# astra-vision/rain-rendering

Measured on AMD Instinct MI355X. Metric: rainy frames/sec @ 1242x375, 100 mm/hr, higher is better.
Workload: dtype f64 alpha/mask, f32 colour

## Files before the change

### rain-rendering_amd/csrc/rainhip.hip

```cpp
#include <hip/hip_runtime.h>

#include <dlfcn.h>

#include <cstddef>
#include <cstdio>
#include <cstdlib>
#include <algorithm>
#include <cstring>
#include <string>
#include <type_traits>
#include <mutex>
#include <unordered_map>
#include <vector>

#include "rainhip.h"
#include "rr_device.h"
#include "rr_prepass.h"
#include "rr_deflate.h"
#include "rr_pngrows.h"
#include "rr_particles.h"
#include "rr_lens.h"

using namespace rr;

// ... 555 lines not shown
    m = wrap ? N + 4 : N;
    int* qx = s_px[wave][g];
    int* qy = s_py[wave][g];
    const int idx = (wrap && k > pp) ? k + 4 : k;
    qx[idx] = ipx;
    qy[idx] = ipy;
    if (wrap && k == pp) {
      const int cols = dm.We, rows = dm.He;
      if (top) {
        qx[pp + 1] = cols; qy[pp + 1] = ipy;
        qx[pp + 2] = cols; qy[pp + 2] = 0;
        qx[pp + 3] = 0;    qy[pp + 3] = 0;
        qx[pp + 4] = 0;    qy[pp + 4] = ipy_next;
      } else {
        qx[pp + 1] = 0;    qy[pp + 1] = ipy;
        qx[pp + 2] = 0;    qy[pp + 2] = rows;
        qx[pp + 3] = cols; qy[pp + 3] = rows;
        qx[pp + 4] = cols; qy[pp + 4] = ipy_next;
      }
    }
  }
  if (ext) {
    const rr_ext_tile e = fr.ext[dg];
    const int np = imin(imax(e.n_poly, 0), POLY_STRIDE);
    bool fine = true;
    for (int v = k; v < np; v += N) {
      const double vx = e.poly_xy[2 * v], vy = e.poly_xy[2 * v + 1];
      fine = fine && fov_coord_ok(vx) && fov_coord_ok(vy);
      s_px[wave][g][v] = (int32_t)vx;
      s_py[wave][g][v] = (int32_t)vy;
    }
    const unsigned long long bad_e = __ballot(!fine) & gmask;
    m = bad_e ? 0 : np;
  }
  wave_lds_sync();
  {
    const int* qx = s_px[wave][imin(g, FOV_GROUPS - 1)];
    const int* qy = s_py[wave][imin(g, FOV_GROUPS - 1)];
    const int x0v = m > 0 ? qx[0] : 0, y0v = m > 0 ? qy[0] : 0;
    int vdif = -1;
    for (int v = k; v < m; v += N)
      if (vdif < 0 && (qx[v] != x0v || qy[v] != y0v)) vdif = v;
    const unsigned long long bd = __ballot(vdif >= 0) & gmask;
    const int va = __shfl(vdif, bd ? __ffsll((long long)bd) - 1 : lane);
    bool nz = false;
    if (bd) {
      const int64_t ax = (int64_t)qx[va] - x0v, ay = (int64_t)qy[va] - y0v;
      for (int v = k; v < m; v += N) nz = nz || (ax * ((int64_t)qy[v] - y0v) - ay * ((int64_t)qx[v] - x0v) != 0);
    }
    if ((__ballot(nz) & gmask) == 0ull) m = 0;
  }
  if (act && k == 0) sc.npts[gi] = m;
  const int He = dm.He;
  int* xl = s_xl[wave];
  int* xr = s_xr[wave];
  uint32_t packed[FOV_GROUPS][NCH];
#pragma unroll
  for (int c = 0; c < NCH; c++) {
    xl[c * 64 + lane] = 1 << 30;
    xr[c * 64 + lane] = -(1 << 30);
#pragma unroll
    for (int k = 0; k < FOV_GROUPS; k++) packed[k][c] = 0;
  }
  for (int gg = 0; gg < G; gg++) {
    const int mg = __builtin_amdgcn_readfirstlane(__shfl(m, gg * N));
    if (mg <= 0) continue;
    const bool cvg = cv_rule && fov_fill_rule_cv_applies(s_px[wave][gg], s_py[wave][gg], mg, N, He, dm.We);
    int cnt = 0;
    if (lane < mg) {
      const int j = (lane + 1 == mg) ? 0 : lane + 1;
      const int x0 = s_px[wave][gg][lane], y0 = s_py[wave][gg][lane], x1 = s_px[wave][gg][j], y1 = s_py[wave][gg][j];
      const bool swp = y1 < y0;
      const int ylo = swp ? y1 : y0, yhi = swp ? y0 : y1;
      const int xa = swp ? x1 : x0, dx = (swp ? x0 : x1) - xa;
      const int den = yhi - ylo;
      const float inv = den > 0 ? 1.0f / (float)(2 * den) : 0.f;
      const int ra = imax(ylo, 0), rb = imin(yhi, He - 1);
      cnt = rb - ra + 1;
      int d16 = 0, q_hh = 0, q_hr = 0;
      if (cvg && den > 0) edge_cv_consts(dx, den, d16, q_hh, q_hr);
      s_edge[wave][3 * lane] = make_int4(ylo, ra, rb, xa);
      s_edge[wave][3 * lane + 1] = make_int4(dx, den, __float_as_int(inv), 0);
      s_edge[wave][3 * lane + 2] = make_int4(d16, q_hh, q_hr, 0);
    }
    wave_lds_sync();
    for (int e = 0; e < mg; e += 2) {
      const int eb = imin(e + 1, mg - 1);
      const int nmax = imax(__builtin_amdgcn_readlane(cnt, e), __builtin_amdgcn_readlane(cnt, eb));
      if (nmax <= 0) continue;
      const int me = lane < 32 ? e : eb;
      const int4 A = s_edge[wave][3 * me], B = s_edge[wave][3 * me + 1], C = s_edge[wave][3 * me + 2];
      const int ylo = A.x, ra = A.y, rbv = A.z, xa = A.w, dx = B.x, den = B.y;
      const float inv = __int_as_float(B.z);
      const bool hz = den == 0;
      const int hz_l = imin(xa, xa + dx), hz_h = imax(xa, xa + dx);
      const int dx2 = 2 * dx, dn = 2 * den;
      for (int c = 0; c < nmax; c += 32) {
        const int y = ra + c + (lane & 31);
        if (y <= rbv) {
          const int t = y - ylo;
          const int n2 = __mul24(dx2, t);
          int q = (int)floorf((float)n2 * inv);
          int rem = n2 - __mul24(q, dn);
          if (rem < 0) { q -= 1; rem += dn; }
          else if (rem >= dn) { q += 1; rem -= dn; }
          int l = xa + q + (rem >= den ? 1 : 0), h = l;
          if (cvg && !hz) edge_row_cv(xa, xa + dx, den, dx, C.x, C.y, C.z, t, q, rem, l, h);
          atomicMin(&xl[y], hz ? hz_l : l);
          atomicMax(&xr[y], hz ? hz_h : h);
        }
      }
    }
    wave_lds_sync();
#pragma unroll
    for (int c = 0; c < NCH; c++) {
      const int y = c * 64 + lane;
      const int a = imax(xl[y], 0), b = imin(xr[y], dm.We - 1);
      xl[y] = 1 << 30;
      xr[y] = -(1 << 30);
      uint32_t v = 0;
      if (y < He && a <= b) v = (uint32_t)a | ((uint32_t)(b + 1) << 16);
#pragma unroll
      for (int k = 0; k < FOV_GROUPS; k++)
        if (k == gg) packed[k][c] = v;
    }
  }
  bool have[FOV_GROUPS];
  int dk[FOV_GROUPS];
  const int col = (from_list && act) ? sc.fov_slot[gi] : dg;
#pragma unroll
  for (int k = 0; k < FOV_GROUPS; k++) {
    have[k] = k < G && __builtin_amdgcn_readfirstlane(__shfl(m, k < G ? k * N : 0)) > 0;
    dk[k] = __builtin_amdgcn_readfirstlane(__shfl(col, k < G ? k * N : 0));
  }
#pragma unroll
  for (int c = 0; c < NCH; c++) {
    const int y = c * 64 + lane;
    if (y < Hp) {
      uint32_t* out = sc.spans + ((int64_t)f * Hp + y) * Dp;
#pragma unroll
      for (int k = 0; k < FOV_GROUPS; k++)
        if (have[k]) out[dk[k]] = packed[k][c];
    }
  }
  if (!from_list) break;
  wave_lds_sync();
  }
}

#ifndef RR_DDA_WAVES
#define RR_DDA_WAVES 1
#endif
constexpr int DDA_WAVES = RR_DDA_WAVES;
template <int CTRL, int ROW_MASK>
__device__ inline int dpp_keep_i32(int v) { return __builtin_amdgcn_update_dpp(v, v, CTRL, ROW_MASK, 0xf, false); }
__device__ inline int wave_min_scan_i32(int v) {
  v = imin(v, dpp_keep_i32<0x111, 0xf>(v));
  v = imin(v, dpp_keep_i32<0x112, 0xf>(v));
  v = imin(v, dpp_keep_i32<0x114, 0xf>(v));
  v = imin(v, dpp_keep_i32<0x118, 0xf>(v));
  v = imin(v, dpp_keep_i32<0x142, 0xa>(v));
  v = imin(v, dpp_keep_i32<0x143, 0xc>(v));
  return v;
}
__device__ inline int wave_max_scan_i32(int v) {
  v = imax(v, dpp_keep_i32<0x111, 0xf>(v));
  v = imax(v, dpp_keep_i32<0x112, 0xf>(v));
  v = imax(v, dpp_keep_i32<0x114, 0xf>(v));
  v = imax(v, dpp_keep_i32<0x118, 0xf>(v));
  v = imax(v, dpp_keep_i32<0x142, 0xa>(v));
  v = imax(v, dpp_keep_i32<0x143, 0xc>(v));
  return v;
}

constexpr uint32_t FOV_KEY_LAST = 0xffffu;
__global__ __launch_bounds__(64 * DDA_WAVES) void k_fov_vertices(const FrameDesc* frames, Dims dm, rr_camera cam, int max_drops, int ordered, Scratch sc) {
  const int f = blockIdx.y, wave = threadIdx.x >> 6, lane = threadIdx.x & 63;
  const FrameDesc& fr = frames[f];
  const int N = cam.n_fov;
  const int i = (blockIdx.x * DDA_WAVES + wave) * 64 + lane;
  const bool act = i < fr.n_drops;
  const int64_t gi = (int64_t)f * max_drops + (act ? i : 0);
  if (fr.strategy == 1) {
    if (act) {
      sc.npts[gi] = -1;
      sc.fov_rec[gi] = make_uint4(0u, 0u, 0u, (ordered ? FOV_KEY_LAST : 0u) << 16);
    }
    return;
  }
  uint32_t* const gpix = sc.fov_pix + (int64_t)f * N * max_drops + (act ? i : 0);
  auto pixv = [&](int kk) -> uint32_t& { return gpix[(int64_t)kk * max_drops]; };
  uint32_t top_xy = 0;
  int uns = 0;
  int count_true = 0, count_false = 0;
  int ktop = 0, ytop = 1 << 30, ybot = -(1 << 30), r_first = 0;
  bool spread = false, on_map = true;
  int turns = 0, dir = 0, dir_first = 0;
  float dist = 0.f;
  if (act) {
    FovSetup32 F;
    const rr_drop d = load_drop(fr.drops + i);
    fov_setup32(d, (float)cam.fov_cos, (float)cam.fov_sin, F, uns);
    dist = sqrtf(F.pos[0] * F.pos[0] + F.pos[1] * F.pos[1] + F.pos[2] * F.pos[2]);
    float az_prev = 0.f, er_prev = 0.f, az0 = 0.f, er0 = 0.f;
    int y_prev = 0, y0v = 0;
    for (int k = 0; k < N; k++) {
      float az, er, pxf, pyf;
      fov_vertex32(F, (float)cam.radius, (float)cam.phi_cos[k], (float)cam.phi_sin[k], dm.He, dm.We, az, er, pxf, pyf, uns);
      const int ix = (int)pxf, iy = (int)pyf;
      const uint32_t vxy = (uint32_t)(ix & 0xffff) | ((uint32_t)(iy & 0xffff) << 16);
      pixv(k) = vxy;
      on_map = on_map && ix >= 0 && ix < dm.We && iy >= 0 && iy < dm.He;
      const int r = imin(imax(iy, 0), dm.He - 1);
      if (k == 0) { az0 = az; er0 = er; r_first = r; y0v = iy; }
      else {
        const bool c = fov_wrap_cnd32(az_prev, az, er_prev, er, uns);
        count_true += c ? 1 : 0;
        count_false += c ? 0 : 1;
        spread = spread || iabs(r - r_first) >= 2;
        const int sg = iy > y_prev ? 1 : (iy < y_prev ? -1 : 0);
        if (sg != 0) {
          if (dir == 0) dir_first = sg;
          else if (sg != dir) turns++;
          dir = sg;
        }
      }
      if (iy < ytop) { ytop = iy; ktop = k; top_xy = vxy; }
      ybot = imax(ybot, iy);
      az_prev = az; er_prev = er; y_prev = iy;
    }
    {
      const bool c = fov_wrap_cnd32(az_prev, az0, er_prev, er0, uns);
      count_true += c ? 1 : 0;
      count_false += c ? 0 : 1;
      const int sg = y0v > y_prev ? 1 : (y0v < y_prev ? -1 : 0);
      if (sg != 0) {
        if (dir != 0 && sg != dir) turns++;
        dir = sg;
      }
      if (dir != 0 && dir_first != 0 && dir != dir_first) turns++;
    }
  }
  if (act) {
    const uint32_t v0 = pixv(0), va = pixv(N / 2);
    const int x0v = (int)(v0 & 0xffffu), y0v = (int)(v0 >> 16), ax = (int)(va & 0xffffu) - x0v, ay = (int)(va >> 16) - y0v;
    bool sure_nc = false;
    for (int k = 1; k < N; k++) {
      const uint32_t v = pixv(k);
      sure_nc = sure_nc || poly_surely_not_collinear_step(ax, ay, (int)(v & 0xffffu) - x0v, (int)(v >> 16) - y0v);
    }
    if (!sure_nc) uns |= 256;
  }
  const bool certain_fail = (uns & 128) && !(uns & 3);
  const bool wrap = count_true == 1 || count_false == 1;
  const bool undecided = (uns & ~128) != 0 || count_true == 0 || count_false == 0 || (!wrap && !spread);
  const bool monotone = turns <= 2;
  const bool mine = act && !certain_fail && !undecided && !wrap && monotone;
  if (act && certain_fail) sc.npts[gi] = 0;
  if (act && !certain_fail && !mine) {
    const int pos = atomicAdd(&sc.fov_list_n[f], 1);
    sc.fov_list[(int64_t)f * max_drops + pos] = i;
  }
  if (mine) sc.npts[gi] = N;
  if (act) {
    uint32_t key = 0u;
    if (ordered) {
      const int bucket = (int)fminf(fmaxf(dist * 4.0f, 0.f), 62.0f);
      key = mine ? ((uint32_t)bucket << 10) | (uint32_t)imin(imax(ytop, 0), 1023) : FOV_KEY_LAST;
    }
    sc.fov_rec[gi] = make_uint4((uint32_t)ytop, (uint32_t)ybot, top_xy, (uint32_t)ktop | (mine ? 256u : 0u) | (on_map ? 512u : 0u) | (key << 16));
  }
}

__global__ __launch_bounds__(64 * DDA_WAVES) void k_fov_dda(const FrameDesc* frames, Dims dm, rr_camera cam, int max_drops, int Hp, int Dp, int cv_rule, Scratch sc) {
  const int f = blockIdx.y, wave = threadIdx.x >> 6, lane = threadIdx.x & 63;
  const FrameDesc& fr = frames[f];
  const int N = cam.n_fov;
  if (fr.strategy == 1) return;
  const int s = (blockIdx.x * DDA_WAVES + wave) * 64 + lane;
  const bool act = s < fr.n_drops;
  const int i = act ? sc.fov_order[(int64_t)f * max_drops + s] : 0;
  const uint4 dr = act ? sc.fov_rec[(int64_t)f * max_drops + i] : make_uint4(0u, 0u, 0u, 0u);
  const bool mine = act && (dr.w & 256u);
  if (__ballot(mine) == 0ull) return;
  const int ytop = (int)dr.x, ybot = (int)dr.y, ktop = (int)(dr.w & 255u);
  const uint32_t top_xy = dr.z;
  uint4* const erec = sc.fov_erec + (int64_t)f * N * max_drops + s;
  const uint32_t* const gpix = sc.fov_pix + (int64_t)f * N * max_drops + i;
  auto pixv = [&](int kk) -> uint32_t { return gpix[(int64_t)kk * max_drops]; };
  const bool cvr = cv_rule && (dr.w & 512u);
  if (mine) {
    const uint32_t vfirst = pixv(0);
    uint32_t va = vfirst;
    for (int k = 0; k < N; k++) {
      const uint32_t vb = k + 1 == N ? vfirst : pixv(k + 1);
      const int x0 = (int)(va & 0xffffu), y0 = (int)(va >> 16), x1 = (int)(vb & 0xffffu), y1 = (int)(vb >> 16);
      const bool swp = y1 < y0;
      uint32_t r[4];
      dda_edge_record(swp ? x1 : x0, swp ? y1 : y0, swp ? x0 : x1, swp ? y0 : y1, cvr, r);
      erec[(int64_t)k * max_drops] = make_uint4(r[0], r[1], r[2], r[3]);
      va = vb;
    }
  }
  auto rec = [&](int kk, uint32_t r[4]) {
    const uint4 v = erec[(int64_t)kk * max_drops];
    r[0] = v.x; r[1] = v.y; r[2] = v.z; r[3] = v.w;
  };
  DdaCursors<decltype(rec)> cur;
  if (mine) cur.init(rec, N, ktop, top_xy);
  uint32_t* out = sc.spans + (int64_t)f * Hp * Dp + s;
  const int wtop = __builtin_amdgcn_readlane(wave_min_scan_i32(mine ? imin(imax(ytop, 0), Hp) : Hp), 63);
  const int wend = imax(__builtin_amdgcn_readlane(wave_max_scan_i32(mine ? imin(imax(ybot + 1, 0), Hp) : 0), 63), wtop);
  for (int y = 0; y < wtop; y++)
    if (mine) out[(int64_t)y * Dp] = 0u;
  for (int y = wtop; y < wend; y++) {
    int lo = 1 << 30, hi = -(1 << 30);
    if (mine && y >= ytop && y <= ybot) cur.row(rec, y, lo, hi);
    const int a = imax(lo, 0), b = imin(hi, dm.We - 1);
    if (mine) out[(int64_t)y * Dp] = (y < dm.He && a <= b) ? ((uint32_t)a | ((uint32_t)(b + 1) << 16)) : 0u;
  }
  for (int y = wend; y < Hp; y++)
    if (mine) out[(int64_t)y * Dp] = 0u;
}

template <int CTRL, int ROW_MASK>
__device__ inline double dpp_move_f64(double v) {
  int lo = __double2loint(v), hi = __double2hiint(v);
  lo = __builtin_amdgcn_update_dpp(0, lo, CTRL, ROW_MASK, 0xf, true);
  hi = __builtin_amdgcn_update_dpp(0, hi, CTRL, ROW_MASK, 0xf, true);
  return __hiloint2double(hi, lo);
}
__device__ inline double row16_incl_scan_f64(double v) {
  v += dpp_move_f64<0x111, 0xf>(v);
  v += dpp_move_f64<0x112, 0xf>(v);
  v += dpp_move_f64<0x114, 0xf>(v);
  v += dpp_move_f64<0x118, 0xf>(v);
  return v;
}
__device__ inline double wave_incl_scan_f64(double v) {
  v = row16_incl_scan_f64(v);
  v += dpp_move_f64<0x142, 0xa>(v);
  v += dpp_move_f64<0x143, 0xc>(v);
  return v;
}
template <int CTRL, int ROW_MASK>
__device__ inline double dpp_keep_f64(double v) {
  int lo = __double2loint(v), hi = __double2hiint(v);
  lo = __builtin_amdgcn_update_dpp(lo, lo, CTRL, ROW_MASK, 0xf, false);
  hi = __builtin_amdgcn_update_dpp(hi, hi, CTRL, ROW_MASK, 0xf, false);
  return __hiloint2double(hi, lo);
}
__device__ inline double wave_min_scan_f64(double v) {
  v = dmin(v, dpp_keep_f64<0x111, 0xf>(v));
  v = dmin(v, dpp_keep_f64<0x112, 0xf>(v));
  v = dmin(v, dpp_keep_f64<0x114, 0xf>(v));
  v = dmin(v, dpp_keep_f64<0x118, 0xf>(v));
  v = dmin(v, dpp_keep_f64<0x142, 0xa>(v));
  v = dmin(v, dpp_keep_f64<0x143, 0xc>(v));
  return v;
}
__device__ inline double wave_max_scan_f64(double v) {
  v = dmax(v, dpp_keep_f64<0x111, 0xf>(v));
  v = dmax(v, dpp_keep_f64<0x112, 0xf>(v));
  v = dmax(v, dpp_keep_f64<0x114, 0xf>(v));
  v = dmax(v, dpp_keep_f64<0x118, 0xf>(v));
  v = dmax(v, dpp_keep_f64<0x142, 0xa>(v));
  v = dmax(v, dpp_keep_f64<0x143, 0xc>(v));
  return v;
}
__device__ inline double readlane_f64(double v, int l) {
  int lo = __double2loint(v), hi = __double2hiint(v);
  lo = __builtin_amdgcn_readlane(lo, l);
  hi = __builtin_amdgcn_readlane(hi, l);
  return __hiloint2double(hi, lo);
}

template <int DPT, int EMAX>
__global__ __launch_bounds__(1024) void k_fov_sums(const FrameDesc* frames, Dims dm, int max_drops, int Hp, int Dp, int rpb, int nchunk, Scratch sc) {
  extern __shared__ __attribute__((aligned(16))) double s_dyn[];
  const int We = dm.We;
  double2* s_P = reinterpret_cast<double2*>(s_dyn);
  double* s_wt = reinterpret_cast<double*>(s_P + (We + 1));
  const int f = blockIdx.y, band = blockIdx.x % COL_PARTS, part = blockIdx.x / COL_PARTS;
  const int half = part & 1, chunk = part >> 1;
  const int NT = blockDim.x, t = threadIdx.x, lane = t & 63, nw = NT >> 6;
  const int wave = __builtin_amdgcn_readfirstlane(t >> 6);
  const FrameDesc& fr = frames[f];
  const int n = fr.n_drops;
  const int per = (n + nchunk - 1) / nchunk;
  const int d0 = chunk * per, d1 = imin(n, d0 + per);
  if (d0 >= n) return;
  const int y0 = band * rpb, y1 = imin(dm.He, y0 + rpb);
  const int Cw = (((We + nw - 1) / nw) + 1) & ~1;
  const int cw0 = wave * Cw;
  const uint32_t* spf = sc.spans + (int64_t)f * Hp * Dp;
  uint32_t sp[DPT];
#pragma unroll
  for (int d = 0; d < DPT; d++) {
    const int i = d0 + d * NT + t;
    sp[d] = (uint32_t)((i < d1 && sc.npts[(int64_t)f * max_drops + i] > 0) ? i : max_drops);
  }
  if (t == 0) s_P[0] = make_double2(0.0, 0.0);
  double S[DPT][2];
  uint32_t any = 0;
#pragma unroll
  for (int d = 0; d < DPT; d++) S[d][0] = S[d][1] = 0.0;
  double tot0 = 0.0, tot1 = 0.0;
  double pa[EMAX][2], pb[EMAX][2];
  const bool e32 = (fr.in_types & RR_IN_ENV_F32) != 0;
  auto load_row = [&](int y) {
    const global_ptr<const double> env = as_global(static_cast<const double*>(fr.env)) + (int64_t)y * We * 3;
    const global_ptr<const double> om = as_global(static_cast<const double*>(fr.omega)) + (int64_t)y * We;
    const global_ptr<const float> envf = as_global(static_cast<const float*>(fr.env)) + (int64_t)y * We * 3;
    const global_ptr<const float> omf = as_global(static_cast<const float*>(fr.omega)) + (int64_t)y * We;
    auto E = [&](int i) { return e32 ? (double)envf[i] : env[i]; };
    auto O = [&](int i) { return e32 ? (double)omf[i] : om[i]; };
#pragma unroll
    for (int e = 0; e < EMAX; e++) {
      const int cl = e * 128 + 2 * lane, c = cw0 + cl;
      pa[e][0] = pa[e][1] = pb[e][0] = pb[e][1] = 0.0;
      if (cl < Cw && c < We) {
        const double w = O(c);
        pa[e][0] = (half ? E(c * 3 + 2) : E(c * 3 + 0)) * w;
        pa[e][1] = half ? w : E(c * 3 + 1) * w;
        if (c + 1 < We) {
          const double w1 = O(c + 1);
          pb[e][0] = (half ? E(c * 3 + 5) : E(c * 3 + 3)) * w1;
          pb[e][1] = half ? w1 : E(c * 3 + 4) * w1;
        }
      }
    }
  };
  if (y0 < y1) load_row(y0);
  for (int yq = y0; yq < y1; yq += 4) {
    uint4 q[DPT];
#pragma unroll
    for (int d = 0; d < DPT; d++)
      q[d] = make_uint4(spf[(int64_t)yq * Dp + sp[d]], spf[(int64_t)(yq + 1) * Dp + sp[d]], spf[(int64_t)(yq + 2) * Dp + sp[d]],
                        spf[(int64_t)(yq + 3) * Dp + sp[d]]);
#pragma unroll
    for (int j = 0; j < 4; j++) {
      const int y = yq + j;
      if (y >= y1) break;
      double carry[2] = {0.0, 0.0};
      double ps[EMAX][2];
#pragma unroll
      for (int e = 0; e < EMAX; e++) {
        if (e * 128 < Cw) {
#pragma unroll
          for (int k = 0; k < 2; k++) {
            const double v = wave_incl_scan_f64(pa[e][k] + pb[e][k]) + carry[k];
            ps[e][k] = v;
            carry[k] = readlane_f64(v, 63);
          }
        }
      }
      if (lane == 0) { s_wt[wave * 2 + 0] = carry[0]; s_wt[wave * 2 + 1] = carry[1]; }
      __syncthreads();
      double basev[2];
#pragma unroll
      for (int k = 0; k < 2; k++) {
        const double wt = row16_incl_scan_f64(lane < nw ? s_wt[lane * 2 + k] : 0.0);
        const double u = readlane_f64(wt, wave > 0 ? wave - 1 : 0);
        basev[k] = wave > 0 ? u : 0.0;
      }
#pragma unroll
      for (int e = 0; e < EMAX; e++) {
        const int cl = e * 128 + 2 * lane, c = cw0 + cl;
        if (cl < Cw && c < We) {
          const double o0 = basev[0] + ps[e][0], o1 = basev[1] + ps[e][1];
          s_P[c + 1] = make_double2(o0 - pb[e][0], o1 - pb[e][1]);
          if (c + 1 < We) s_P[c + 2] = make_double2(o0, o1);
// ... 7270 lines not shown
```

### rain-rendering_amd/csrc/rr_device.h

```cpp
#pragma once
#include <math.h>
#include <stdint.h>

#include "rainhip.h"

#if defined(__HIPCC__)
#include <hip/hip_runtime.h>
#define RR_HD __host__ __device__ inline
#else
#define RR_HD inline
#endif

#if defined(__clang__)
#pragma clang fp contract(off)
#endif

namespace rr {

enum { KIND_BIG = 0, KIND_ROT = 1, KIND_EXT = 2 };
enum { RS_AREA = 0, RS_AREA_FAST = 1, RS_LINEAR = 2 };

struct Dims {
  int32_t H, W, He, We;
};
// ... 684 lines not shown
    fov_vertex32(F, (float)cam.radius, (float)cam.phi_cos[k], (float)cam.phi_sin[k], He, We, azs[k], ers[k], ptx[k], pty[k], unsure);
  azs[N] = azs[0];
  ers[N] = ers[0];
  int count_true = 0, count_false = 0, pos_true = -1, pos_false = -1;
  for (int k = 0; k < N; k++) {
    bool cnd = fov_wrap_cnd32(azs[k], azs[k + 1], ers[k], ers[k + 1], unsure);
    if (cnd) { count_true++; if (pos_true < 0) pos_true = k; }
    else { count_false++; if (pos_false < 0) pos_false = k; }
  }
  int m = 0;
  if ((unsure & 128) && !(unsure & (1 | 2))) {
    if (used32) *used32 = 1;
    return 0;
  }
  if (!unsure && pos_true >= 0 && pos_false >= 0) {
    const bool wrap = count_true == 1 || count_false == 1, top = count_true == 1;
    const int pp = top ? pos_true : pos_false;
    const int rows = He, cols = We;
    for (int k = 0; k < N; k++) {
      px[m] = (int32_t)ptx[k]; py[m] = (int32_t)pty[k]; m++;
      if (wrap && k == pp) {
        const int nxt = (pp + 1) % N;
        if (top) {
          px[m] = cols; py[m] = (int32_t)pty[pp]; m++;
          px[m] = cols; py[m] = 0; m++;
          px[m] = 0; py[m] = 0; m++;
          px[m] = 0; py[m] = (int32_t)pty[nxt]; m++;
        } else {
          px[m] = 0; py[m] = (int32_t)pty[pp]; m++;
          px[m] = 0; py[m] = rows; m++;
          px[m] = cols; py[m] = rows; m++;
          px[m] = cols; py[m] = (int32_t)pty[nxt]; m++;
        }
      }
    }
    if (!wrap) {
      const int r0 = imin(imax((int)pty[0], 0), He - 1);
      bool spread = false;
      for (int k = 1; k < N; k++) spread = spread || iabs(imin(imax((int)pty[k], 0), He - 1) - r0) >= 2;
      if (!spread) unsure |= 32;
    }
    if (!poly_surely_not_collinear(px, py, m)) unsure |= 256;
  } else {
    unsure |= 64;
  }
  if (used32) *used32 = unsure ? -unsure : 1;
  if (unsure) return fov_polygon(d, cam, He, We, px, py);
  return m;
}

RR_HD bool fov_rowspan(const int32_t* px, const int32_t* py, int n, int y, int We, int& xl, int& xr) {
  int lo = 1 << 30, hi = -(1 << 30);
  for (int i = 0; i < n; i++) {
    int j = (i + 1 == n) ? 0 : i + 1;
    int x0 = px[i], y0 = py[i], x1 = px[j], y1 = py[j];
    int ylo = imin(y0, y1), yhi = imax(y0, y1);
    if (y < ylo || y > yhi) continue;
    if (y0 == y1) {
      lo = imin(lo, imin(x0, x1));
      hi = imax(hi, imax(x0, x1));
    } else {
      int xa, yA, xb, yB;
      if (y1 < y0) { xa = x1; yA = y1; xb = x0; yB = y0; } else { xa = x0; yA = y0; xb = x1; yB = y1; }
      int64_t den = yB - yA;
      int64_t num = (int64_t)(xb - xa) * (int64_t)(y - yA);
      int64_t nn = 2 * num + den, dn = 2 * den;
      int64_t q = nn / dn;
      if ((nn % dn != 0) && ((nn < 0) != (dn < 0))) q -= 1;
      int xv = xa + (int)q;
      lo = imin(lo, xv);
      hi = imax(hi, xv);
    }
  }
  xl = imax(lo, 0);
  xr = imin(hi, We - 1);
  return xl <= xr;
}

RR_HD bool fov_fill_rule_cv_applies(const int32_t* px, const int32_t* py, int n, int n_fov, int He, int We);
RR_HD bool fov_rowspan_cv(const int32_t* px, const int32_t* py, int n, int y, int We, int& xl, int& xr) {
  int lo = 1 << 30, hi = -(1 << 30);
  for (int i = 0; i < n; i++) {
    const int j = (i + 1 == n) ? 0 : i + 1;
    const int x0 = px[i], y0 = py[i], x1 = px[j], y1 = py[j];
    if (y < imin(y0, y1) || y > imax(y0, y1)) continue;
    if (y0 == y1) {
      lo = imin(lo, imin(x0, x1));
      hi = imax(hi, imax(x0, x1));
      continue;
    }
    const bool swp = y1 < y0;
    const int xa = swp ? x1 : x0, ya = swp ? y1 : y0, xb = swp ? x0 : x1, yb = swp ? y0 : y1;
    const int den = yb - ya, dn = 2 * den, dx = xb - xa, dxa = iabs(dx), t = y - ya;
    const int64_t N2 = (int64_t)2 * dx * t;
    int64_t Q = N2 / dn;
    if (N2 % dn != 0 && N2 < 0) Q -= 1;
    const int R = (int)(N2 - Q * dn);
    int l, h_;
    if (den > dxa) {
      l = h_ = xa + (int)Q + (R >= den + 1 ? 1 : 0);
    } else {
      const int hh = dxa / dn, hr = dxa - hh * dn;
      l = xa + (int)Q - hh + (R >= hr ? 1 : 0);
      h_ = xa + (int)Q + hh + (R + hr >= dn ? 1 : 0);
      l = imax(l, imin(xa, xb));
      h_ = imin(h_, imax(xa, xb));
    }
    lo = imin(lo, l);
    hi = imax(hi, h_);
    if (t < den) {
      const int64_t num = ((int64_t)dx << 17) + den;
      const int64_t dx16 = num / dn;
      const int s = (int)((((int64_t)xa << 16) + (int64_t)t * dx16 + 32768) >> 16);
      lo = imin(lo, s);
      hi = imax(hi, s);
    }
  }
  xl = imax(lo, 0);
  xr = imin(hi, We - 1);
  return xl <= xr;
}

RR_HD void edge_cv_consts(int dx, int den, int& dx16, int& hh, int& hr) {
  const int dn = 2 * den, dxa = iabs(dx);
  const int num = dx * 131072 + den;
  dx16 = num / dn;
  hh = dxa / dn;
  hr = dxa - hh * dn;
}
RR_HD void edge_row_cv(int xa, int xb, int den, int dx, int dx16, int hh, int hr, int t, int Q, int R, int& l, int& h) {
  const int dn = 2 * den;
  if (den > iabs(dx)) {
    l = h = xa + Q + (R >= den + 1 ? 1 : 0);
  } else {
    l = xa + Q - hh + (R >= hr ? 1 : 0);
    h = xa + Q + hh + (R + hr >= dn ? 1 : 0);
    l = imax(l, imin(xa, xb));
    h = imin(h, imax(xa, xb));
  }
  if (t < den) {
    const int s = xa + ((t * dx16 + 32768) >> 16);
    l = imin(l, s);
    h = imax(h, s);
  }
}

RR_HD int mul24i(int a, int b) {
#if defined(__HIP_DEVICE_COMPILE__)
  return __mul24(a, b);
#else
  return a * b;
#endif
}
struct DdaSide {
  int xa, xb, yb, kv;
  int mn, mx;
  int Q, R, W;
  int dn, hh, tl, th, qs, rs, d16, wk;
  uint32_t n_r0, n_r1, n_r2, n_r3;
};
RR_HD void dda_take_edge(DdaSide& S, int xa, int ya, int xb, int yb, uint32_t w0, uint32_t w1) {
  S.xa = xa;
  S.xb = xb;
  S.yb = yb;
  S.mn = imin(xa, xb);
  S.mx = imax(xa, xb);
  const int den = yb - ya, dx = xb - xa;
  S.dn = 2 * den;
  S.Q = 0;
  S.R = 0;
  S.W = 32768;
  S.d16 = (int)w0;
  S.wk = (int)((w1 >> 23) & 1u);
  S.hh = (int)(w1 & 0x7ffu);
  S.tl = (int)((w1 >> 11) & 0x7ffu);
  S.th = ((w1 >> 22) & 1u) ? S.tl : S.dn - S.tl;
  S.qs = S.d16 >> 16;
  S.rs = 2 * dx - mul24i(S.qs, S.dn);
}
RR_HD void dda_pixels(const DdaSide& S, int y, int& x0, int& x1) {
  const int base = S.xa + S.Q;
  x0 = imax(base - S.hh + (S.R >= S.tl ? 1 : 0), S.mn);
  x1 = imin(base + S.hh + (S.R >= S.th ? 1 : 0), S.mx);
  if (S.wk && y < S.yb) {
    const int sx = S.xa + (S.W >> 16);
    x0 = imin(x0, sx);
    x1 = imax(x1, sx);
  }
  if (S.dn == 0) {
    x0 = S.mn;
    x1 = S.mx;
  }
}
RR_HD void dda_edge_record(int xu, int yu, int xl, int yl, bool cv, uint32_t r[4]) {
  const int den = yl - yu, dx = xl - xu;
  r[0] = r[1] = 0u;
  if (den > 0) {
    int dx16, hh, hr;
    edge_cv_consts(dx, den, dx16, hh, hr);
    r[0] = (uint32_t)dx16;
    if (!cv) r[1] = 0u | ((uint32_t)den << 11) | (1u << 22);
    else if (den > iabs(dx)) r[1] = 0u | ((uint32_t)(den + 1) << 11) | (1u << 22) | (1u << 23);
    else r[1] = (uint32_t)hh | ((uint32_t)hr << 11) | (1u << 23);
  }
  DdaSide S;
  dda_take_edge(S, xu, yu, xl, yl, r[0], r[1]);
  int x0, x1;
  dda_pixels(S, yu, x0, x1);
  r[2] = (uint32_t)(x0 & 0xffff) | ((uint32_t)(x1 & 0xffff) << 16);
  r[3] = (uint32_t)(xl & 0xffff) | ((uint32_t)(yl & 0xffff) << 16);
  if (den <= 0) r[0] = (uint32_t)(xu & 0xffff);
}
template <class E>
struct DdaCursors {
  DdaSide s0, s1;
  int used, N;
  template <int C>
  RR_HD static int next_k(int k, int n) { return C == 0 ? (k + 1 == n ? 0 : k + 1) : (k == 0 ? n - 1 : k - 1); }
  template <int C>
  RR_HD void fetch(DdaSide& S, const E& rec) const {
    uint32_t r[4];
    rec(C == 0 ? S.kv : next_k<C>(S.kv, N), r);
    S.n_r0 = r[0]; S.n_r1 = r[1]; S.n_r2 = r[2]; S.n_r3 = r[3];
  }
  template <int C, bool STEP>
  RR_HD void advance_edge(DdaSide& S, const E& rec, int& lo, int& hi) const {
    const int xa = S.xb, ya = S.yb;
    uint32_t w0 = S.n_r0;
    const uint32_t w1 = S.n_r1, w2 = S.n_r2, w3 = S.n_r3;
    S.kv = next_k<C>(S.kv, N);
    fetch<C>(S, rec);
    int xe = (int)(w3 & 0xffffu);
    const int ye = (int)(w3 >> 16);
    if (ye == ya) {
      if (C == 1) xe = (int)w0;
      w0 = 0u;
    }
    dda_take_edge(S, xa, ya, xe, ye, w0, w1);
    if (STEP) {
      lo = imin(lo, (int)(w2 & 0xffffu));
      hi = imax(hi, (int)(w2 >> 16));
      if (S.dn > 0) {
        const int carry = S.rs >= S.dn ? 1 : 0;
        S.R = S.rs - (carry ? S.dn : 0);
        S.Q = S.qs + carry;
        S.W = 32768 + S.d16;
      }
    }
  }
  template <int C>
  RR_HD void init_side(DdaSide& S, const E& rec, int ktop, uint32_t top_xy) const {
    S.xb = (int)(top_xy & 0xffffu);
    S.yb = (int)(top_xy >> 16);
    S.kv = ktop;
    fetch<C>(S, rec);
    int lo = 0, hi = 0;
    advance_edge<C, false>(S, rec, lo, hi);
  }
  RR_HD void init(const E& rec, int n, int ktop, uint32_t top_xy) {
    N = n;
    used = 2;
    init_side<0>(s0, rec, ktop, top_xy);
    init_side<1>(s1, rec, ktop, top_xy);
  }
  RR_HD static void step(DdaSide& S) {
    const int r = S.R + S.rs;
    const int carry = r >= S.dn ? 1 : 0;
    S.R = r - (carry ? S.dn : 0);
    S.Q += S.qs + carry;
    S.W += S.d16;
  }
  template <int C>
  RR_HD void side_row(DdaSide& S, const E& rec, int y, int& lo, int& hi) {
    {
      int x0, x1;
      dda_pixels(S, y, x0, x1);
      lo = imin(lo, x0);
      hi = imax(hi, x1);
    }
    step(S);
    while (y == S.yb && used < N) {
      used++;
      advance_edge<C, true>(S, rec, lo, hi);
    }
  }
  RR_HD void row(const E& rec, int y, int& lo, int& hi) {
    lo = 1 << 30;
    hi = -(1 << 30);
    side_row<0>(s0, rec, y, lo, hi);
    side_row<1>(s1, rec, y, lo, hi);
  }
};

RR_HD int poly_row_turns(const int32_t* py, int n) {
  int turns = 0, dir = 0, dir_first = 0;
  for (int k = 1; k <= n; k++) {
    const int a = py[k - 1], b = py[k == n ? 0 : k];
    const int sg = b > a ? 1 : (b < a ? -1 : 0);
    if (sg != 0) {
      if (dir == 0) dir_first = sg;
      else if (sg != dir) turns++;
      dir = sg;
    }
  }
  if (dir != 0 && dir_first != 0 && dir != dir_first) turns++;
  return turns;
}

RR_HD bool fov_fill_rule_cv_applies(const int32_t* px, const int32_t* py, int n, int n_fov, int He, int We) {
  if (n != n_fov || n < 3) return false;
  for (int k = 0; k < n; k++)
    if (px[k] < 0 || px[k] >= We || py[k] < 0 || py[k] >= He) return false;
  return poly_row_turns(py, n) <= 2;
}

RR_HD void colour_from_sums(const double S[4], double sum_omega, double ambient, double Kbgr[3]) {
  double x = S[0] / S[3], y = S[1] / S[3];
  double avg_fov_lum = S[2] / sum_omega;
  double drop_Y = 0.94 * avg_fov_lum + 0.06 * ambient;
  double Yg = ((0.31 + 0.8124) + 0.01) / 0.17697 * drop_Y;
  double X = (Yg * x) / y;
  double Z = (Yg * (1 - x - y)) / y;
  double r = (X * 0.41847 + Yg * -0.091169) + Z * 0.0009209;
  double g = (X * -0.15866 + Yg * 0.25243) + Z * -0.0025498;
  double b = (X * -0.082835 + Yg * 0.015708) + Z * 0.1786;
  Kbgr[0] = b;
  Kbgr[1] = g;
  Kbgr[2] = r;
}

RR_HD void solve8(double A[8][8], double b[8], double x[8]) {
#pragma unroll
  for (int col = 0; col < 8; col++) {
    int piv = col;
    double best = fabs(A[col][col]);
#pragma unroll
    for (int r = col + 1; r < 8; r++)
      if (fabs(A[r][col]) > best) { best = fabs(A[r][col]); piv = r; }
#pragma unroll
    for (int r = col + 1; r < 8; r++)
      if (r == piv) {
#pragma unroll
        for (int c = 0; c < 8; c++) { double t = A[col][c]; A[col][c] = A[r][c]; A[r][c] = t; }
        double t = b[col]; b[col] = b[r]; b[r] = t;
      }
#pragma unroll
    for (int r = col + 1; r < 8; r++) {
      double f = A[r][col] / A[col][col];
#pragma unroll
      for (int c = col + 1; c < 8; c++) A[r][c] = A[r][c] - f * A[col][c];
      b[r] = b[r] - f * b[col];
    }
  }
#pragma unroll
  for (int r = 7; r >= 0; r--) {
    double s = b[r];
#pragma unroll
    for (int c = r + 1; c < 8; c++) s = s - A[r][c] * x[c];
    x[r] = s / A[r][r];
  }
}

RR_HD void invert3(const double m[9], double t[9]) {
  double d = m[0] * (m[4] * m[8] - m[5] * m[7]) - m[1] * (m[3] * m[8] - m[5] * m[6]) + m[2] * (m[3] * m[7] - m[4] * m[6]);
  if (d == 0.0 || !(fabs(d) < 1.7e308)) {
    for (int i = 0; i < 9; i++) t[i] = 0.0;
    return;
  }
  d = 1.0 / d;
  t[0] = (m[4] * m[8] - m[5] * m[7]) * d;
  t[1] = (m[2] * m[7] - m[1] * m[8]) * d;
  t[2] = (m[1] * m[5] - m[2] * m[4]) * d;
  t[3] = (m[5] * m[6] - m[3] * m[8]) * d;
  t[4] = (m[0] * m[8] - m[2] * m[6]) * d;
  t[5] = (m[2] * m[3] - m[0] * m[5]) * d;
  t[6] = (m[3] * m[7] - m[4] * m[6]) * d;
  t[7] = (m[1] * m[6] - m[0] * m[7]) * d;
  t[8] = (m[0] * m[4] - m[1] * m[3]) * d;
}

RR_HD int py_slice_index(int i, int n) {
  if (i < 0) { i += n; if (i < 0) i = 0; }
  else if (i > n) i = n;
  return i;
}

RR_HD void raw_tile_key(const rr_drop& d, const DropPlan& p, uint32_t key[8]) {
  for (int k = 0; k < 8; k++) key[k] = 0u;
  key[0] = 0xffffffffu;
  if (p.status != RR_DROP_OK || (p.kind != KIND_BIG && p.kind != KIND_ROT)) return;
  if (p.tw < 0 || p.tw > 65535 || p.th < 0 || p.th > 65535) return;
  if (p.kind == KIND_BIG) {
    const double d0 = floor(d.iw1), d1 = floor(d.iw2);
    if (!(d0 > -2.0e9 && d0 < 2.0e9 && d1 > -2.0e9 && d1 < 2.0e9)) return;
    const int minx = imax(imin(d.x0, d.x1), 0), miny = imax(imin(d.y0, d.y1), 0);
    key[2] = (uint32_t)(d.x0 - minx);
    key[3] = (uint32_t)(d.y0 - miny);
    key[4] = (uint32_t)(d.x1 - minx);
    key[5] = (uint32_t)(d.y1 - miny);
    key[6] = (uint32_t)(int32_t)d0;
    key[7] = (uint32_t)(int32_t)d1;
  } else {
    uint64_t a, b;
    const double al = d.rot_cos, be = d.rot_sin;
    __builtin_memcpy(&a, &al, 8);
    __builtin_memcpy(&b, &be, 8);
    key[2] = (uint32_t)a; key[3] = (uint32_t)(a >> 32);
    key[4] = (uint32_t)b; key[5] = (uint32_t)(b >> 32);
  }
  key[0] = (uint32_t)p.kind | ((uint32_t)(p.flip & 1) << 4) | ((uint32_t)p.tex << 8);
  key[1] = (uint32_t)p.tw | ((uint32_t)p.th << 16);
}

RR_HD void plan_big_homography(const rr_drop& d, int sw, int sh, double mi[9]) {
  const double d0 = floor(d.iw1), d1 = floor(d.iw2);
  const int minx = imax(imin(d.x0, d.x1), 0), miny = imax(imin(d.y0, d.y1), 0);
  float src[4][2] = {{0.f, 0.f}, {(float)sw, 0.f}, {(float)sw, (float)sh}, {0.f, (float)sh}};
  float dst[4][2];
  dst[0][0] = (float)(d.x0 - minx);                        dst[0][1] = (float)(d.y0 - miny);
  dst[1][0] = (float)((double)(d.x0 - minx) + d0);         dst[1][1] = (float)(d.y0 - miny);
  dst[2][0] = (float)(((double)(d.x1 - minx) + d1) + 0.001); dst[2][1] = (float)(d.y1 - miny);
  dst[3][0] = (float)((double)(d.x1 - minx) + 0.001);      dst[3][1] = (float)(d.y1 - miny);
  double A[8][8], bb[8], xx[8];
#pragma unroll
  for (int i = 0; i < 8; i++)
#pragma unroll
    for (int j = 0; j < 8; j++) A[i][j] = 0.0;
#pragma unroll
  for (int i = 0; i < 4; i++) {
    double sx = src[i][0], sy = src[i][1], ddx = dst[i][0], ddy = dst[i][1];
    A[i][0] = A[i + 4][3] = sx;
    A[i][1] = A[i + 4][4] = sy;
    A[i][2] = A[i + 4][5] = 1.0;
    A[i][6] = -sx * ddx;
    A[i][7] = -sy * ddx;
    A[i + 4][6] = -sx * ddy;
    A[i + 4][7] = -sy * ddy;
    bb[i] = ddx;
    bb[i + 4] = ddy;
  }
  solve8(A, bb, xx);
  double M[9] = {xx[0], xx[1], xx[2], xx[3], xx[4], xx[5], xx[6], xx[7], 1.0};
  invert3(M, mi);
// ... 258 lines not shown
```

Measured before the change: 19130.

## Batch vertex loads and prefetch edge records in FOV DDA rasterization

Loads polygon vertex pixels in batches of 20 registers before processing, in both the collinearity test and the edge-record build loop, so global loads overlap. DdaCursors now prefetches the next edge record right after consuming the current one, with a sched_barrier and inline-asm register pinning, and row handling is split into a per-side pixel step plus a shared vertex-advance branch. The span loop computes 4 rows at a time before storing. This is meant to hide global-memory latency in the DDA kernel, at the cost of extra register pressure and redundant clamped loads on the tail of each batch.

```diff
diff --git a/rain-rendering_amd/csrc/rainhip.hip b/rain-rendering_amd/csrc/rainhip.hip
--- a/rain-rendering_amd/csrc/rainhip.hip
+++ b/rain-rendering_amd/csrc/rainhip.hip
@@ -731,6 +731,11 @@
 #define RR_DDA_WAVES 1
 #endif
 constexpr int DDA_WAVES = RR_DDA_WAVES;
+#ifndef RR_DDA_BLOCK
+#define RR_DDA_BLOCK 4
+#endif
+constexpr int DDA_BLOCK = RR_DDA_BLOCK;
+constexpr int DDA_PIX = 20;
 template <int CTRL, int ROW_MASK>
 __device__ inline int dpp_keep_i32(int v) { return __builtin_amdgcn_update_dpp(v, v, CTRL, ROW_MASK, 0xf, false); }
 __device__ inline int wave_min_scan_i32(int v) {
@@ -824,9 +829,13 @@
     const uint32_t v0 = pixv(0), va = pixv(N / 2);
     const int x0v = (int)(v0 & 0xffffu), y0v = (int)(v0 >> 16), ax = (int)(va & 0xffffu) - x0v, ay = (int)(va >> 16) - y0v;
     bool sure_nc = false;
-    for (int k = 1; k < N; k++) {
-      const uint32_t v = pixv(k);
-      sure_nc = sure_nc || poly_surely_not_collinear_step(ax, ay, (int)(v & 0xffffu) - x0v, (int)(v >> 16) - y0v);
+    for (int k0 = 1; k0 < N; k0 += DDA_PIX) {
+      uint32_t q[DDA_PIX];
+#pragma unroll
+      for (int j = 0; j < DDA_PIX; j++) q[j] = pixv(imin(k0 + j, N - 1));
+#pragma unroll
+      for (int j = 0; j < DDA_PIX; j++)
+        sure_nc = sure_nc || poly_surely_not_collinear_step(ax, ay, (int)(q[j] & 0xffffu) - x0v, (int)(q[j] >> 16) - y0v);
     }
     if (!sure_nc) uns |= 256;
   }
@@ -869,16 +878,26 @@
   auto pixv = [&](int kk) -> uint32_t { return gpix[(int64_t)kk * max_drops]; };
   const bool cvr = cv_rule && (dr.w & 512u);
   if (mine) {
-    const uint32_t vfirst = pixv(0);
-    uint32_t va = vfirst;
-    for (int k = 0; k < N; k++) {
-      const uint32_t vb = k + 1 == N ? vfirst : pixv(k + 1);
-      const int x0 = (int)(va & 0xffffu), y0 = (int)(va >> 16), x1 = (int)(vb & 0xffffu), y1 = (int)(vb >> 16);
-      const bool swp = y1 < y0;
-      uint32_t r[4];
-      dda_edge_record(swp ? x1 : x0, swp ? y1 : y0, swp ? x0 : x1, swp ? y0 : y1, cvr, r);
-      erec[(int64_t)k * max_drops] = make_uint4(r[0], r[1], r[2], r[3]);
-      va = vb;
+    uint32_t q[DDA_PIX + 1];
+    q[0] = pixv(0);
+    for (int k0 = 0; k0 < N; k0 += DDA_PIX) {
+#pragma unroll
+      for (int j = 0; j < DDA_PIX; j++) {
+        const int kn = k0 + 1 + j;
+        q[1 + j] = pixv(kn < N ? kn : 0);
+      }
+      const int k1 = imin(k0 + DDA_PIX, N);
+#pragma nounroll
+      for (int k = k0; k < k1; k++) {
+        const uint32_t va = q[0], vb = q[1];
+        const int x0 = (int)(va & 0xffffu), y0 = (int)(va >> 16), x1 = (int)(vb & 0xffffu), y1 = (int)(vb >> 16);
+        const bool swp = y1 < y0;
+        uint32_t r[4];
+        dda_edge_record(swp ? x1 : x0, swp ? y1 : y0, swp ? x0 : x1, swp ? y0 : y1, cvr, r);
+        erec[(int64_t)k * max_drops] = make_uint4(r[0], r[1], r[2], r[3]);
+#pragma unroll
+        for (int j = 0; j < DDA_PIX; j++) q[j] = q[j + 1];
+      }
     }
   }
   auto rec = [&](int kk, uint32_t r[4]) {
@@ -892,11 +911,26 @@
   const int wend = imax(__builtin_amdgcn_readlane(wave_max_scan_i32(mine ? imin(imax(ybot + 1, 0), Hp) : 0), 63), wtop);
   for (int y = 0; y < wtop; y++)
     if (mine) out[(int64_t)y * Dp] = 0u;
-  for (int y = wtop; y < wend; y++) {
+  auto span = [&](int y) -> uint32_t {
     int lo = 1 << 30, hi = -(1 << 30);
     if (mine && y >= ytop && y <= ybot) cur.row(rec, y, lo, hi);
     const int a = imax(lo, 0), b = imin(hi, dm.We - 1);
-    if (mine) out[(int64_t)y * Dp] = (y < dm.He && a <= b) ? ((uint32_t)a | ((uint32_t)(b + 1) << 16)) : 0u;
+    return (y < dm.He && a <= b) ? ((uint32_t)a | ((uint32_t)(b + 1) << 16)) : 0u;
+  };
+  int y = wtop;
+  for (; y + DDA_BLOCK <= wend; y += DDA_BLOCK) {
+    uint32_t buf[DDA_BLOCK];
+#pragma unroll
+    for (int j = 0; j < DDA_BLOCK; j++) buf[j] = span(y + j);
+    if (mine) {
+#pragma unroll
+      for (int j = 0; j < DDA_BLOCK; j++) out[(int64_t)(y + j) * Dp] = buf[j];
+    }
+  }
+#pragma nounroll
+  for (; y < wend; y++) {
+    const uint32_t v = span(y);
+    if (mine) out[(int64_t)y * Dp] = v;
   }
   for (int y = wend; y < Hp; y++)
     if (mine) out[(int64_t)y * Dp] = 0u;
diff --git a/rain-rendering_amd/csrc/rr_device.h b/rain-rendering_amd/csrc/rr_device.h
--- a/rain-rendering_amd/csrc/rr_device.h
+++ b/rain-rendering_amd/csrc/rr_device.h
@@ -860,12 +860,22 @@
   return a * b;
 #endif
 }
+typedef uint32_t DdaRecord __attribute__((vector_size(16)));
+RR_HD uint32_t dda_own(uint32_t w) {
+#if defined(__HIP_DEVICE_COMPILE__)
+  uint32_t r;
+  asm("v_mov_b32 %0, %1" : "=v"(r) : "v"(w));
+  return r;
+#else
+  return w;
+#endif
+}
 struct DdaSide {
   int xa, xb, yb, kv;
   int mn, mx;
   int Q, R, W;
   int dn, hh, tl, th, qs, rs, d16, wk;
-  uint32_t n_r0, n_r1, n_r2, n_r3;
+  DdaRecord n_r;
 };
 RR_HD void dda_take_edge(DdaSide& S, int xa, int ya, int xb, int yb, uint32_t w0, uint32_t w1) {
   S.xa = xa;
@@ -929,15 +939,13 @@
   RR_HD void fetch(DdaSide& S, const E& rec) const {
     uint32_t r[4];
     rec(C == 0 ? S.kv : next_k<C>(S.kv, N), r);
-    S.n_r0 = r[0]; S.n_r1 = r[1]; S.n_r2 = r[2]; S.n_r3 = r[3];
+    S.n_r = DdaRecord{r[0], r[1], r[2], r[3]};
   }
   template <int C, bool STEP>
   RR_HD void advance_edge(DdaSide& S, const E& rec, int& lo, int& hi) const {
     const int xa = S.xb, ya = S.yb;
-    uint32_t w0 = S.n_r0;
-    const uint32_t w1 = S.n_r1, w2 = S.n_r2, w3 = S.n_r3;
-    S.kv = next_k<C>(S.kv, N);
-    fetch<C>(S, rec);
+    uint32_t w0 = dda_own(S.n_r[0]);
+    const uint32_t w1 = dda_own(S.n_r[1]), w2 = S.n_r[2], w3 = S.n_r[3];
     int xe = (int)(w3 & 0xffffu);
     const int ye = (int)(w3 >> 16);
     if (ye == ya) {
@@ -955,21 +963,28 @@
         S.W = 32768 + S.d16;
       }
     }
-  }
-  template <int C>
-  RR_HD void init_side(DdaSide& S, const E& rec, int ktop, uint32_t top_xy) const {
-    S.xb = (int)(top_xy & 0xffffu);
-    S.yb = (int)(top_xy >> 16);
-    S.kv = ktop;
+#if defined(__HIP_DEVICE_COMPILE__)
+    __builtin_amdgcn_sched_barrier(0);
+#endif
+    S.kv = next_k<C>(S.kv, N);
     fetch<C>(S, rec);
-    int lo = 0, hi = 0;
-    advance_edge<C, false>(S, rec, lo, hi);
+  }
+  RR_HD void settle() const {
+#if defined(__HIP_DEVICE_COMPILE__)
+    asm volatile("" ::"v"(s0.n_r), "v"(s1.n_r));
+#endif
   }
   RR_HD void init(const E& rec, int n, int ktop, uint32_t top_xy) {
     N = n;
     used = 2;
-    init_side<0>(s0, rec, ktop, top_xy);
-    init_side<1>(s1, rec, ktop, top_xy);
+    s0.xb = s1.xb = (int)(top_xy & 0xffffu);
+    s0.yb = s1.yb = (int)(top_xy >> 16);
+    s0.kv = s1.kv = ktop;
+    fetch<0>(s0, rec);
+    fetch<1>(s1, rec);
+    int lo = 0, hi = 0;
+    advance_edge<0, false>(s0, rec, lo, hi);
+    advance_edge<1, false>(s1, rec, lo, hi);
   }
   RR_HD static void step(DdaSide& S) {
     const int r = S.R + S.rs;
@@ -979,14 +994,17 @@
     S.W += S.d16;
   }
   template <int C>
-  RR_HD void side_row(DdaSide& S, const E& rec, int y, int& lo, int& hi) {
-    {
-      int x0, x1;
-      dda_pixels(S, y, x0, x1);
-      lo = imin(lo, x0);
-      hi = imax(hi, x1);
-    }
+  RR_HD void side_pixels(DdaSide& S, int y, int& lo, int& hi) const {
+    int x0, x1;
+    dda_pixels(S, y, x0, x1);
+    lo = imin(lo, x0);
+    hi = imax(hi, x1);
     step(S);
+  }
+  template <int C>
+  RR_HD void side_vertex(DdaSide& S, const E& rec, int y, int& lo, int& hi) {
+    used++;
+    advance_edge<C, true>(S, rec, lo, hi);
     while (y == S.yb && used < N) {
       used++;
       advance_edge<C, true>(S, rec, lo, hi);
@@ -995,8 +1013,13 @@
   RR_HD void row(const E& rec, int y, int& lo, int& hi) {
     lo = 1 << 30;
     hi = -(1 << 30);
-    side_row<0>(s0, rec, y, lo, hi);
-    side_row<1>(s1, rec, y, lo, hi);
+    side_pixels<0>(s0, y, lo, hi);
+    side_pixels<1>(s1, y, lo, hi);
+    if ((y == s0.yb || y == s1.yb) && used < N) {
+      settle();
+      if (y == s0.yb) side_vertex<0>(s0, rec, y, lo, hi);
+      if (y == s1.yb && used < N) side_vertex<1>(s1, rec, y, lo, hi);
+    }
   }
 };
 
```

After: 19290 (median of 6 runs). No clear change (+0.8%).
